# url-kaist/Quatro

Hardware: NVIDIA H100
Metric: registrations/sec (64-ring pair) (higher is better)
Workload: dtype f32 (front end, match, graph filter) / f64 (graph boundary, GNC, COTE)

## Files before the change

### quatro_b200/csrc/api.cu

```cuda
#include <new>
#include <stddef.h>
#include <stdio.h>
#include <stdlib.h>
#include <string.h>
#include <map>
#include <mutex>
#include <utility>

#include "handle.cuh"

using namespace qb;

namespace {

__global__ void wave_init_kernel(int* ctr_block, int n_ints, int* bbox, int n_clouds) {
  const int i = blockIdx.x * blockDim.x + threadIdx.x;
  if (i < n_ints) ctr_block[i] = 0;
  if (i < n_clouds * 6) bbox[i] = (i % 6) < 3 ? INT_MAX : INT_MIN;
}

__global__ void cache_copy_kernel(int to_cache, const int* __restrict__ slot_of_cloud, int V, float4* __restrict__ w_vox, float4* __restrict__ w_nrm,
                                  float* __restrict__ w_desc, int* __restrict__ w_n, int* __restrict__ w_status, float4* __restrict__ c_vox,
                                  float4* __restrict__ c_nrm, float* __restrict__ c_desc, int* __restrict__ c_n, int* __restrict__ c_status) {
  const int cloud = blockIdx.z, slot = slot_of_cloud[cloud], row = blockIdx.y;
  const int q = blockIdx.x * blockDim.x + threadIdx.x;
  if (slot < 0) return;
  const int n = to_cache ? w_n[cloud] : c_n[slot];
  if (row == 42) {
    if (q == 0) {
      if (to_cache) { c_n[slot] = w_n[cloud]; c_status[slot] = w_status[cloud]; }
      else { w_n[cloud] = c_n[slot]; w_status[cloud] = c_status[slot]; }
    }
    return;
  }
  if (q >= n || q >= V) return;
  if (row < kDescK) {
    float* w = w_desc + ((size_t)cloud * kDescK + row) * V + q;
    float* c = c_desc + ((size_t)slot * kDescK + row) * V + q;
    if (to_cache) *c = *w; else *w = *c;
  } else if (row == 40) {
    if (to_cache) c_vox[(size_t)slot * V + q] = w_vox[(size_t)cloud * V + q]; else w_vox[(size_t)cloud * V + q] = c_vox[(size_t)slot * V + q];
  } else {
    if (to_cache) c_nrm[(size_t)slot * V + q] = w_nrm[(size_t)cloud * V + q]; else w_nrm[(size_t)cloud * V + q] = c_nrm[(size_t)slot * V + q];
  }
}

size_t carve_counters(int* base, size_t S, WaveCounters* c) {
  const size_t C = 2 * S;
  size_t n = 0;
  auto take = [&](size_t k) {
    int* p = base ? base + n : nullptr;
    n += k;
    return p;
  };
  c->n_edges = reinterpret_cast<long long*>(take(2 * S));
  c->n_valid = take(C);
  c->n_vox = take(C);
  c->n_lat = take(C);
  c->n_cells = take(C);
  c->cloud_status = take(C);
  c->bbox = take(C * 6);
  c->vox_digits = take(C);
  c->n_mutual = take(S);
  c->n_corr = take(S);
  c->swapped = take(S);
  c->n_clique = take(S);
  c->max_core = take(S);
  c->n_final = take(S);
  c->flags = take(S);
  return n + 2;
}

int lane_alloc(const Lane& like, std::unique_ptr<Lane>* out) {
  std::unique_ptr<Lane> L(new (std::nothrow) Lane());
  if (!L) return QB200_ERR_CUDA;
  L->S = like.S; L->R = like.R; L->V = like.V; L->Lc = like.Lc; L->W = like.W; L->NS = like.NS;
  L->device = like.device; L->n_sm = like.n_sm; L->force_exact_match = like.force_exact_match; L->err = like.err;
  L->tc_verify = like.tc_verify; L->tc_prof = like.tc_prof;
  QB_CUDA_TRY(L, L->own_stream.create(cudaStreamNonBlocking));
  L->stream = L->own_stream;
  const size_t S = L->S, R = L->R, V = L->V, Lc = L->Lc, W = L->W, C = 2 * S;
  QB_CUDA_TRY(L, L->d_cloud_ptr.alloc(C));
  QB_CUDA_TRY(L, L->d_cloud_n.alloc(C));
  QB_CUDA_TRY(L, L->d_raw_off.alloc(C + 1));
  QB_CUDA_TRY(L, L->h_cloud_ptr.alloc(C));
  QB_CUDA_TRY(L, L->h_cloud_n.alloc(C));
  QB_CUDA_TRY(L, L->h_raw_off.alloc(C + 1));
  QB_CUDA_TRY(L, L->raw_stage.alloc(C * R));
  const size_t n_sort = C * (R > V ? R : V) + 64;
  const size_t n_hist = C * 256 * ((R + kVsTile - 1) / kVsTile);
  QB_CUDA_TRY(L, L->key_a.alloc(n_sort));
  QB_CUDA_TRY(L, L->key_b.alloc(n_sort));
  QB_CUDA_TRY(L, L->val_a.alloc(n_sort > n_hist ? n_sort : n_hist));
  QB_CUDA_TRY(L, L->val_b.alloc(n_sort));
  QB_CUDA_TRY(L, L->aos_scratch.alloc(2 * V * kDescDim));
  L->cub_bytes = sort_temp_bytes((int)(C * V));
  QB_CUDA_TRY(L, L->cub_temp.alloc_bytes(L->cub_bytes));
  QB_CUDA_TRY(L, L->vox_start.alloc(C * (V + 1)));
  QB_CUDA_TRY(L, L->vox_pts.alloc(C * V));
  QB_CUDA_TRY(L, L->cell_key.alloc(C * V));
  QB_CUDA_TRY(L, L->cell_start.alloc(C * (V + 1)));
  QB_CUDA_TRY(L, L->normals.alloc(C * V));
  QB_CUDA_TRY(L, L->spfh.alloc(C * V * kDescPad));
  QB_CUDA_TRY(L, L->nbr_list.alloc(C * kNbrGlobalCap * V));
  QB_CUDA_TRY(L, L->nbr_cnt.alloc(C * V));
  QB_CUDA_TRY(L, L->desc_t.alloc(C * kDescK * V));
  QB_CUDA_TRY(L, cudaMemset(L->desc_t, 0, C * kDescK * V * sizeof(float)));
  QB_CUDA_TRY(L, L->desc_tiles.alloc(C * kDescK * V * 3));
  QB_CUDA_TRY(L, cudaMemset(L->desc_tiles, 0, C * kDescK * V * 3 * sizeof(float)));
  QB_CUDA_TRY(L, L->desc_norm.alloc(C * V));
  QB_CUDA_TRY(L, L->tc_fallback.alloc(S));
  QB_CUDA_TRY(L, L->tc_stats.alloc(32));
  QB_CUDA_TRY(L, cudaMemset(L->tc_stats, 0, 32 * sizeof(unsigned long long)));
  QB_CUDA_TRY(L, L->rowbest.alloc(S * V));
  QB_CUDA_TRY(L, L->colpart.alloc(L->colpart_count()));
  QB_CUDA_TRY(L, L->colbest.alloc(S * V));
  QB_CUDA_TRY(L, L->mut_i.alloc(S * V));
  QB_CUDA_TRY(L, L->mut_j.alloc(S * V));
  QB_CUDA_TRY(L, L->mark.alloc(S * V));
  QB_CUDA_TRY(L, L->partner.alloc(S * V));
  QB_CUDA_TRY(L, L->mean.alloc(C * 4));
  QB_CUDA_TRY(L, L->corr_src.alloc(S * Lc));
  QB_CUDA_TRY(L, L->corr_tgt.alloc(S * Lc));
  QB_CUDA_TRY(L, L->ma.alloc(S * Lc));
  QB_CUDA_TRY(L, L->mb.alloc(S * Lc));
  QB_CUDA_TRY(L, L->adj.alloc(S * Lc * W));
  QB_CUDA_TRY(L, L->adjp.alloc(S * Lc * W));
  QB_CUDA_TRY(L, L->deg.alloc(S * Lc));
  QB_CUDA_TRY(L, L->kcore.alloc(S * (Lc + 2)));
  QB_CUDA_TRY(L, L->korder.alloc(S * (Lc + 2)));
  QB_CUDA_TRY(L, L->rank_of.alloc(S * (Lc + 2)));
  QB_CUDA_TRY(L, L->by_rank.alloc(S * (Lc + 2)));
  QB_CUDA_TRY(L, L->kbin.alloc(S * (Lc + 2)));
  QB_CUDA_TRY(L, L->clique.alloc(S * Lc));
  QB_CUDA_TRY(L, L->final_inl.alloc(S * Lc));
  QB_CUDA_TRY(L, L->rot_mask.alloc(S * Lc));
  QB_CUDA_TRY(L, L->trans_mask.alloc(S * Lc));
  QB_CUDA_TRY(L, L->d_solve.alloc(S));
  QB_CUDA_TRY(L, L->h_solve.alloc(S));
  QB_CUDA_TRY(L, L->d_front.alloc(C));
  QB_CUDA_TRY(L, L->h_front.alloc(C));
  if (Lc > (size_t)kKcoreSmemVerts) {
    QB_CUDA_TRY(L, L->kcore_ws.alloc(S * kcore_ws_bytes((int)Lc)));
    QB_CUDA_TRY(L, L->chain_ws.alloc(S * kCliqueWarps * Lc));
  }
  if (Lc > (size_t)kPoseSmemClique) QB_CUDA_TRY(L, L->pose_ws.alloc(S * pose_ws_bytes((int)Lc)));
  QB_CUDA_TRY(L, L->d_results.alloc(S));
  QB_CUDA_TRY(L, cudaMemset(L->d_results, 0, S * sizeof(qb200_result)));
  QB_CUDA_TRY(L, L->h_results.alloc(S));
  L->ctr_ints = carve_counters(nullptr, S, &L->ctr);
  QB_CUDA_TRY(L, L->ctr_block.alloc(L->ctr_ints));
  QB_CUDA_TRY(L, L->hctr_block.alloc(L->ctr_ints));
  carve_counters(L->ctr_block, S, &L->ctr);
  carve_counters(L->hctr_block, S, &L->hctr);
  for (Event& e : L->ev) QB_CUDA_TRY(L, e.create());
  for (Event& e : L->kev) QB_CUDA_TRY(L, e.create());
  QB_CUDA_TRY(L, cudaStreamSynchronize(L->stream));
  *out = std::move(L);
  return QB200_OK;
}

void reset_timers(qb200_handle* h) {
  memset(h->stage_ms, 0, sizeof(h->stage_ms));
  memset(h->kernel_ms, 0, sizeof(h->kernel_ms));
  memset(h->kernel_calls, 0, sizeof(h->kernel_calls));
}

}

namespace qb {
cudaError_t ensure_dyn_smem(int device, const void* kernel, size_t bytes) {
  static std::mutex mu;
  static std::map<std::pair<const void*, int>, size_t> current;
  std::lock_guard<std::mutex> lock(mu);
  size_t& cur = current[std::make_pair(kernel, device)];
  if (bytes > cur) {
    const cudaError_t e = cudaFuncSetAttribute(kernel, cudaFuncAttributeMaxDynamicSharedMemorySize, (int)bytes);
// ... 810 lines not shown
```

### quatro_b200/csrc/common.cuh

```cuda
#pragma once
#include <cuda_runtime.h>
#include <stdint.h>
#include <stdio.h>

#include "quatro_b200.h"

namespace qb {

constexpr int kOffIJ = 1 << 17;
constexpr int kOffK = 1 << 15;
constexpr uint64_t kCellMask = (1ull << 52) - 1;
constexpr uint64_t kCellInvalid = kCellMask;
constexpr int kCloudShift = 52;

__host__ __device__ __forceinline__ bool cell_ok(int i, int j, int k) {
  return i >= -kOffIJ && i < kOffIJ - 1 && j >= -kOffIJ && j < kOffIJ - 1 && k >= -kOffK && k < kOffK - 1;
}
__host__ __device__ __forceinline__ uint64_t cell_key(int i, int j, int k) {
  return ((uint64_t)(k + kOffK) << 36) | ((uint64_t)(j + kOffIJ) << 18) | (uint64_t)(i + kOffIJ);
}

constexpr int kVoxShift = 31;
constexpr uint64_t kVoxMask = (1ull << kVoxShift) - 1;
constexpr uint64_t kVoxInvalid = kVoxMask;
constexpr int kVsChunks = 64;
constexpr int kVsTile = 2048;

__device__ __forceinline__ bool raw_point_kept(const float4 p, int skip_flagged) {
  return isfinite(p.x) && isfinite(p.y) && isfinite(p.z) && !(skip_flagged && p.w < 0.0f);
}
__host__ __device__ __forceinline__ int vox_chunk_size(int n) { return n > 0 ? (n + kVsChunks - 1) / kVsChunks : 1; }

constexpr int kDescDim = 33;
constexpr int kDescPad = 36;
constexpr int kDescK = 40;
constexpr int kMatchTile = 128;
constexpr int kNbrGlobalCap = 80;

struct WaveCounters {
  int* n_valid;
  int* n_vox;
  int* n_lat;
  int* n_cells;
  int* cloud_status;
  int* bbox;
  int* vox_digits;
  int* n_mutual;
  int* n_corr;
  int* swapped;
  int* n_clique;
  int* max_core;
  int* n_final;
  int* flags;
  long long* n_edges;
};

#define QB_CUDA_TRY(h, expr)                                                                    \
  do {                                                                                          \
    cudaError_t _e = (expr);                                                                    \
    if (_e != cudaSuccess) {                                                                    \
      (h)->fail(__FILE__, __LINE__, cudaGetErrorString(_e));                                    \
      return QB200_ERR_CUDA;                                                                    \
    }                                                                                           \
  } while (0)

__device__ __forceinline__ int float_ordered(float f) {
  const int i = __float_as_int(f);
  return i >= 0 ? i : i ^ 0x7FFFFFFF;
}
__host__ __device__ __forceinline__ float ordered_float(int i) {
  const int j = i >= 0 ? i : i ^ 0x7FFFFFFF;
#ifdef __CUDA_ARCH__
  return __int_as_float(j);
#else
  float f;
  memcpy(&f, &j, 4);
  return f;
#endif
}

__host__ __device__ __forceinline__ bool vox_product_exceeds(long long a, long long b, long long c) {
  const long long lim = 2147483647LL;
  if (a > lim || b > lim || c > lim) return true;
  const long long ab = a * b;
  return ab > lim || ab * c > lim;
}
__device__ __forceinline__ bool vox_axis(int omin, int omax, float inv_leaf, long long* span, long long* min_b, long long* div_b) {
  const float mn = ordered_float(omin), mx = ordered_float(omax);
  const float lo = floorf(mn * inv_leaf), hi = floorf(mx * inv_leaf);
  if (!(lo >= -2147483648.0f && hi < 2147483648.0f)) return false;
  const float s = (mx - mn) * inv_leaf;
  if (!(s < 2147483648.0f)) return false;
  *span = (long long)s + 1;
  *min_b = (long long)lo;
  *div_b = (long long)hi - *min_b + 1;
  return true;
}
__device__ __forceinline__ bool vox_grid(const int* __restrict__ bbox, float inv_leaf, long long* min_b, long long* div_b) {
  long long t0, t1, t2;
  if (!vox_axis(bbox[0], bbox[3], inv_leaf, &t0, &min_b[0], &div_b[0]) || !vox_axis(bbox[1], bbox[4], inv_leaf, &t1, &min_b[1], &div_b[1]) ||
      !vox_axis(bbox[2], bbox[5], inv_leaf, &t2, &min_b[2], &div_b[2]))
    return false;
  return !vox_product_exceeds(t0, t1, t2) && !vox_product_exceeds(div_b[0], div_b[1], div_b[2]);
}

__device__ __forceinline__ int vox_digits(const int* __restrict__ bbox, int n_valid, float inv_leaf) {
  if (n_valid <= 0) return 0;
  long long m[3], d[3];
  if (!vox_grid(bbox, inv_leaf, m, d)) return -1;
// ... 40 lines not shown
```

### quatro_b200/csrc/frontend.cu

```cuda
#include <cub/device/device_radix_sort.cuh>
#include <type_traits>

#include "fpfh_math.cuh"
#include "handle.cuh"

namespace qb {

size_t sort_temp_bytes(int max_items) {
  size_t bytes = 0;
  cub::DeviceRadixSort::SortPairs(nullptr, bytes, (const uint64_t*)nullptr, (uint64_t*)nullptr, (const uint32_t*)nullptr,
                                  (uint32_t*)nullptr, max_items, 0, 64, (cudaStream_t)0);
  return bytes;
}

int sort_pairs(Lane* h, int n_items, int end_bit) {
  if (n_items <= 0) return QB200_OK;
  size_t bytes = h->cub_bytes;
  QB_CUDA_TRY(h, cub::DeviceRadixSort::SortPairs(h->cub_temp.get(), bytes, h->key_a.get(), h->key_b.get(), h->val_a.get(), h->val_b.get(), n_items, 0, end_bit,
                                                 h->stream));
  h->launches += 1 + (end_bit + 7) / 8;
  return QB200_OK;
}

static int clog2(int n) {
  int b = 0;
  while ((1 << b) < n) ++b;
  return b;
}


__global__ void __launch_bounds__(256) voxel_bbox_kernel(const float4* const* __restrict__ cloud_ptr, const int* __restrict__ cloud_n,
                                                         const CloudFront* __restrict__ front, int* __restrict__ bbox,
                                                         int* __restrict__ n_valid, int* __restrict__ chunk_cnt) {
  const int cloud = blockIdx.y;
  const int n = cloud_n[cloud];
  const int skip_flagged = front[cloud].skip_flagged;
  const float4* __restrict__ pts = cloud_ptr[cloud];
  int mn0 = INT_MAX, mn1 = INT_MAX, mn2 = INT_MAX, mx0 = INT_MIN, mx1 = INT_MIN, mx2 = INT_MIN, cnt = 0;
  constexpr int kInFlight = 8;
  __shared__ int s_cc[kVsChunks];
  if (threadIdx.x < kVsChunks) s_cc[threadIdx.x] = 0;
  __syncthreads();
  const int cs = vox_chunk_size(n);
  const int per_cta = kVsChunks / gridDim.x;
  for (int cl = 0; cl < per_cta; ++cl) {
    const int ch = blockIdx.x * per_cta + cl;
    const int c0 = ch * cs, c1 = min(n, c0 + cs);
    int ccnt = 0;
    for (int i0 = c0 + threadIdx.x; i0 < c1; i0 += kInFlight * 256) {
      float4 pp[kInFlight];
#pragma unroll
      for (int j = 0; j < kInFlight; ++j) pp[j] = i0 + j * 256 < c1 ? __ldg(pts + i0 + j * 256) : make_float4(NAN, NAN, NAN, 0.f);
#pragma unroll
      for (int j = 0; j < kInFlight; ++j) {
        const float4 p = pp[j];
        if (i0 + j * 256 >= c1 || !raw_point_kept(p, skip_flagged)) continue;
        const int ox = float_ordered(p.x), oy = float_ordered(p.y), oz = float_ordered(p.z);
        mn0 = min(mn0, ox); mn1 = min(mn1, oy); mn2 = min(mn2, oz);
        mx0 = max(mx0, ox); mx1 = max(mx1, oy); mx2 = max(mx2, oz);
        ++ccnt;
      }
    }
    cnt += ccnt;
    ccnt = __reduce_add_sync(0xffffffffu, ccnt);
    if (lane_id() == 0 && ccnt) atomicAdd(&s_cc[ch], ccnt);
  }
  __syncthreads();
  if ((int)threadIdx.x < per_cta) chunk_cnt[cloud * kVsChunks + blockIdx.x * per_cta + threadIdx.x] = s_cc[blockIdx.x * per_cta + threadIdx.x];
#pragma unroll
  for (int o = 16; o > 0; o >>= 1) {
    mn0 = min(mn0, __shfl_xor_sync(0xffffffffu, mn0, o)); mn1 = min(mn1, __shfl_xor_sync(0xffffffffu, mn1, o));
    mn2 = min(mn2, __shfl_xor_sync(0xffffffffu, mn2, o)); mx0 = max(mx0, __shfl_xor_sync(0xffffffffu, mx0, o));
    mx1 = max(mx1, __shfl_xor_sync(0xffffffffu, mx1, o)); mx2 = max(mx2, __shfl_xor_sync(0xffffffffu, mx2, o));
    cnt += __shfl_xor_sync(0xffffffffu, cnt, o);
  }
  __shared__ int s_red[7];
  if (threadIdx.x == 0) { s_red[0] = s_red[1] = s_red[2] = INT_MAX; s_red[3] = s_red[4] = s_red[5] = INT_MIN; s_red[6] = 0; }
  __syncthreads();
  if (lane_id() == 0 && cnt) {
    atomicMin(&s_red[0], mn0); atomicMin(&s_red[1], mn1); atomicMin(&s_red[2], mn2);
    atomicMax(&s_red[3], mx0); atomicMax(&s_red[4], mx1); atomicMax(&s_red[5], mx2);
    atomicAdd(&s_red[6], cnt);
  }
  __syncthreads();
  if (threadIdx.x == 0 && s_red[6]) {
    int* b = bbox + cloud * 6;
    atomicMin(b + 0, s_red[0]); atomicMin(b + 1, s_red[1]); atomicMin(b + 2, s_red[2]);
    atomicMax(b + 3, s_red[3]); atomicMax(b + 4, s_red[4]); atomicMax(b + 5, s_red[5]);
    atomicAdd(n_valid + cloud, s_red[6]);
  }
}

__global__ void __launch_bounds__(1024) run_heads_kernel(int mode, const uint64_t* keys, const uint64_t* keys_b, const int* __restrict__ seg_off,
                                                         int V, int key_shift, const CloudFront* __restrict__ front, const int* __restrict__ bbox,
                                                         const int* __restrict__ n_valid_in, int* __restrict__ starts,
                                                         uint64_t* __restrict__ cell_keys, int* __restrict__ n_out, int* __restrict__ n_valid_out,
                                                         int* __restrict__ cloud_status, int* __restrict__ digits_out) {
  __shared__ int sm[33];
  __shared__ int s_overflow, s_valid;
  const int cloud = blockIdx.x;
  const int off = mode == 0 ? seg_off[cloud] : cloud * V;
  const int n = mode == 0 ? n_valid_in[cloud] : V;
  const int digits = mode == 0 ? vox_digits(bbox + cloud * 6, n, front[cloud].inv_leaf) : 0;
  if (digits & 1) keys = keys_b;
  if (threadIdx.x == 0) {
    s_overflow = digits < 0 ? 1 : 0;
    s_valid = 0;
    if (digits_out) digits_out[cloud] = digits;
  }
  __syncthreads();
  if (s_overflow) {
    if (threadIdx.x == 0) {
      n_out[cloud] = 0;
      cloud_status[cloud] = QB200_ERR_VOXEL_OVERFLOW;
      starts[(size_t)cloud * (V + 1)] = 0;
    }
    return;
  }
// ... 412 lines not shown
__global__ void __launch_bounds__(kNbrThreads) fpfh_rare_kernel(const float4* __restrict__ pts, const int* __restrict__ n_pts, int V,
                                                                const uint64_t* __restrict__ cell_key, const int* __restrict__ cell_start,
                                                                const uint32_t* __restrict__ order, const int* __restrict__ n_cells,
                                                                const CloudFront* __restrict__ front, const float* __restrict__ spfh,
                                                                const int* __restrict__ nbr_cnt, float* __restrict__ desc_t) {
  const int cloud = blockIdx.y;
  const int q = blockIdx.x * blockDim.x + threadIdx.x;
  if (q >= n_pts[cloud]) return;
  if (nbr_cnt[(size_t)cloud * V + q] <= kNbrGlobalCap) return;
  const int m = front[cloud].mf;
  const float r2 = front[cloud].rf2;
  const LatticeView L = make_view(cloud, V, pts, cell_key, cell_start, order, n_cells, front[cloud].inv_cell);
  const float4* __restrict__ sp = reinterpret_cast<const float4*>(spfh + (size_t)cloud * V * kDescPad);
  const float4 pq = L.pts[q];
  float o[kDescDim];
#pragma unroll
  for (int b = 0; b < kDescDim; ++b) o[b] = 0.0f;
  double s0 = 0.0, s1 = 0.0, s2 = 0.0;
  for_each_neighbor<false>(L, pq, m, r2, [&](int p, float d2, const float4) {
    if (d2 == 0.0f) return;
    const float weight = 1.0f / d2;
    float s[kDescPad];
#pragma unroll
    for (int v4 = 0; v4 < kDescPad / 4; ++v4) {
      const float4 t = __ldg(sp + (size_t)p * (kDescPad / 4) + v4);
      s[4 * v4] = t.x; s[4 * v4 + 1] = t.y; s[4 * v4 + 2] = t.z; s[4 * v4 + 3] = t.w;
    }
#pragma unroll
    for (int b = 0; b < 11; ++b) { const float v = s[b] * weight; s0 += v; o[b] += v; }
#pragma unroll
    for (int b = 0; b < 11; ++b) { const float v = s[12 + b] * weight; s1 += v; o[11 + b] += v; }
#pragma unroll
    for (int b = 0; b < 11; ++b) { const float v = s[24 + b] * weight; s2 += v; o[22 + b] += v; }
  });
  if (s0 != 0.0) s0 = 100.0 / s0;
  if (s1 != 0.0) s1 = 100.0 / s1;
  if (s2 != 0.0) s2 = 100.0 / s2;
  const float g0 = (float)s0, g1 = (float)s1, g2 = (float)s2;
  float* __restrict__ out = desc_t + (size_t)cloud * kDescK * V + q;
#pragma unroll
  for (int b = 0; b < 11; ++b) out[(size_t)b * V] = o[b] * g0;
#pragma unroll
  for (int b = 11; b < 22; ++b) out[(size_t)b * V] = o[b] * g1;
#pragma unroll
  for (int b = 22; b < 33; ++b) out[(size_t)b * V] = o[b] * g2;
}

__global__ void desc_to_aos_kernel(const float* __restrict__ desc_t, int V, int n, float* __restrict__ out) {
  const int i = blockIdx.x * blockDim.x + threadIdx.x;
  if (i >= n * kDescDim) return;
  const int q = i / kDescDim, d = i % kDescDim;
  out[i] = desc_t[(size_t)d * V + q];
}
__global__ void desc_from_aos_kernel(const float* __restrict__ in, int V, int n, float* __restrict__ desc_t) {
  const int i = blockIdx.x * blockDim.x + threadIdx.x;
  if (i >= n * kDescDim) return;
  const int q = i / kDescDim, d = i % kDescDim;
  desc_t[(size_t)d * V + q] = in[i];
}

void front_voxel(CloudFront* e, float leaf, int skip_flagged) {
  e->inv_leaf = 1.0f / leaf;
  e->skip_flagged = skip_flagged;
}

void front_lattice(CloudFront* e, float normal_radius, float fpfh_radius, float cell) {
  e->inv_cell = 1.0f / cell;
  e->mn = (int)ceilf(normal_radius * e->inv_cell + 1e-3f);
  e->mf = (int)ceilf(fpfh_radius * e->inv_cell + 1e-3f);
  e->rn2 = (float)((double)normal_radius * (double)normal_radius);
  e->rf2 = (float)((double)fpfh_radius * (double)fpfh_radius);
  e->list_usable = (e->mn <= e->mf && e->rn2 <= e->rf2) ? 1 : 0;
}

int upload_front(Lane* L, int n) {
  QB_CUDA_TRY(L, cudaMemcpyAsync(L->d_front, L->h_front, (size_t)n * sizeof(CloudFront), cudaMemcpyHostToDevice, L->stream));
  return QB200_OK;
}

int launch_voxel(Lane* h, int n_clouds) {
  if (n_clouds <= 0) return QB200_OK;
  const dim3 gb(n_clouds >= 16 ? 16 : 64, n_clouds);
  int* chunk_cnt = reinterpret_cast<int*>(h->val_b.get());
  voxel_bbox_kernel<<<gb, 256, 0, h->stream>>>(h->d_cloud_ptr, h->d_cloud_n, h->d_front, h->ctr.bbox, h->ctr.n_valid, chunk_cnt);
  h->launches += 1;
  const int idx_bits = clog2(h->R > 2 ? h->R : 2);
  if (int rc = launch_voxel_sort(h, n_clouds, idx_bits)) return rc;
  run_heads_kernel<<<n_clouds, 1024, 0, h->stream>>>(0, h->key_a, h->key_b, h->d_raw_off, h->V, idx_bits, h->d_front, h->ctr.bbox, h->ctr.n_valid,
                                                     h->vox_start, nullptr, h->ctr.n_vox, nullptr, h->ctr.cloud_status, h->ctr.vox_digits);
  const dim3 gc((h->V + 127) / 128, n_clouds);
  voxel_centroid_kernel<<<gc, 128, 0, h->stream>>>(h->d_cloud_ptr, h->d_raw_off, h->key_a, h->key_b, h->ctr.vox_digits,
                                                   (1ull << idx_bits) - 1, h->vox_start, h->ctr.n_vox, h->V, h->vox_pts);
  h->launches += 2;
  QB_CUDA_TRY(h, cudaGetLastError());
  return QB200_OK;
}

int launch_fpfh(Lane* h, int n_clouds) {
  if (n_clouds <= 0) return QB200_OK;
  const int V = h->V;
  const dim3 gl((V + 255) / 256, n_clouds);
  lattice_keys_kernel<<<gl, 256, 0, h->stream>>>(h->vox_pts, h->ctr.n_vox, V, h->d_front, h->key_a, h->val_a);
  h->launches++;
  int rc = launch_cloud_sort(h, n_clouds, h->ctr.n_vox, 18, 36);
  if (rc == QB200_ERR_UNSUPPORTED) rc = sort_pairs(h, n_clouds * V, kCloudShift + clog2(n_clouds > 1 ? n_clouds : 2));
  if (rc) return rc;
  run_heads_kernel<<<n_clouds, 1024, 0, h->stream>>>(1, h->key_b, nullptr, nullptr, V, 0, nullptr, nullptr, nullptr, h->cell_start, h->cell_key,
                                                     h->ctr.n_cells, h->ctr.n_lat, h->ctr.cloud_status, nullptr);
  const dim3 gp((V + 127) / 128, n_clouds);
  nbr_list_kernel<<<gp, kNbrThreads, 0, h->stream>>>(h->vox_pts, h->ctr.n_vox, V, h->cell_key, h->cell_start, h->val_b, h->ctr.n_cells,
                                                     h->d_front, h->nbr_list, h->nbr_cnt);
  normals_kernel<<<gp, 128, 0, h->stream>>>(h->vox_pts, h->ctr.n_vox, V, h->cell_key, h->cell_start, h->val_b, h->ctr.n_cells, h->d_front,
                                            h->nbr_list, h->nbr_cnt, h->normals);
  spfh_kernel<false><<<gp, kSpfhThreads, 0, h->stream>>>(h->vox_pts, h->normals, h->ctr.n_vox, V, h->cell_key, h->cell_start, h->val_b,
                                                         h->ctr.n_cells, h->d_front, h->spfh, h->nbr_list, h->nbr_cnt);
  spfh_kernel<true><<<gp, kSpfhThreads, 0, h->stream>>>(h->vox_pts, h->normals, h->ctr.n_vox, V, h->cell_key, h->cell_start, h->val_b,
                                                        h->ctr.n_cells, h->d_front, h->spfh, h->nbr_list, h->nbr_cnt);
  fpfh_list_kernel<<<gp, 3 * kNbrThreads, 0, h->stream>>>(h->vox_pts, h->ctr.n_vox, V, h->spfh, h->nbr_list, h->nbr_cnt, h->desc_t);
  fpfh_rare_kernel<<<gp, kNbrThreads, 0, h->stream>>>(h->vox_pts, h->ctr.n_vox, V, h->cell_key, h->cell_start, h->val_b, h->ctr.n_cells,
                                                      h->d_front, h->spfh, h->nbr_cnt, h->desc_t);
  h->launches += 3;
  h->launches += 4;
  QB_CUDA_TRY(h, cudaGetLastError());
  return QB200_OK;
}

int launch_desc_to_aos(Lane* h, int cloud, int n, float* d_out33) {
  if (n <= 0) return QB200_OK;
  desc_to_aos_kernel<<<(n * kDescDim + 255) / 256, 256, 0, h->stream>>>(h->desc_t + (size_t)cloud * kDescK * h->V, h->V, n, d_out33);
  h->launches++;
  QB_CUDA_TRY(h, cudaGetLastError());
  return QB200_OK;
}
int desc_to_aos_rows(Lane* h, const float* desc_rows, int n, float* d_out33) {
  if (n <= 0) return QB200_OK;
  desc_to_aos_kernel<<<(n * kDescDim + 255) / 256, 256, 0, h->stream>>>(desc_rows, h->V, n, d_out33);
  h->launches++;
  QB_CUDA_TRY(h, cudaGetLastError());
  return QB200_OK;
}
int launch_desc_from_aos(Lane* h, int cloud, int n, const float* d_in33) {
  if (n <= 0) return QB200_OK;
  desc_from_aos_kernel<<<(n * kDescDim + 255) / 256, 256, 0, h->stream>>>(d_in33, h->V, n, h->desc_t + (size_t)cloud * kDescK * h->V);
  h->launches++;
  QB_CUDA_TRY(h, cudaGetLastError());
  return QB200_OK;
}

}
```

### quatro_b200/csrc/voxsort.cu

```cuda
#include "handle.cuh"

namespace qb {

constexpr int kVsThreads = 256;

__global__ void __launch_bounds__(kVsThreads) voxel_pack_kernel(const float4* const* __restrict__ cloud_ptr, const int* __restrict__ cloud_n,
                                                                const int* __restrict__ raw_off, const CloudFront* __restrict__ front,
                                                                const int* __restrict__ bbox, const int* __restrict__ n_valid,
                                                                const int* __restrict__ chunk_cnt, int idx_bits, uint64_t* __restrict__ items) {
  __shared__ int sm[33];
  const int cloud = blockIdx.y, chunk = blockIdx.x, tid = threadIdx.x;
  const int n = cloud_n[cloud], off = raw_off[cloud];
  const int cs = vox_chunk_size(n);
  const int c0 = chunk * cs, c1 = min(n, c0 + cs);
  if (c0 >= n) return;
  const float4* __restrict__ pts = cloud_ptr[cloud];
  const float inv_leaf = front[cloud].inv_leaf;
  const int skip_flagged = front[cloud].skip_flagged;
  long long m[3] = {0, 0, 0}, d[3] = {1, 1, 1};
  const bool grid_ok = n_valid[cloud] > 0 && vox_grid(bbox + cloud * 6, inv_leaf, m, d);
  int base = 0;
  {
    int v = 0;
    for (int k = tid; k < chunk; k += kVsThreads) v += chunk_cnt[cloud * kVsChunks + k];
    int tot;
    block_excl_scan(v, sm, &tot);
    base = tot;
  }
  constexpr int kPer = 4;
  for (int r0 = c0; r0 < c1; r0 += kPer * kVsThreads) {
    const int i0 = r0 + kPer * tid;
    uint64_t it[kPer];
    int keep[kPer], nk = 0;
#pragma unroll
    for (int j = 0; j < kPer; ++j) {
      const int i = i0 + j;
      keep[j] = 0; it[j] = 0;
      if (i < c1) {
        const float4 p = __ldg(pts + i);
        if (raw_point_kept(p, skip_flagged)) {
          uint64_t cell = kVoxInvalid;
          if (grid_ok) {
            const int ci = (int)floorf(p.x * inv_leaf), cj = (int)floorf(p.y * inv_leaf), ck = (int)floorf(p.z * inv_leaf);
            cell = (uint64_t)(((long long)ci - m[0]) + ((long long)cj - m[1]) * d[0] + ((long long)ck - m[2]) * d[0] * d[1]);
          }
          it[j] = (cell << idx_bits) | (uint64_t)i;
          keep[j] = 1;
        }
      }
      nk += keep[j];
    }
    int tot;
    int pos = base + block_excl_scan(nk, sm, &tot);
#pragma unroll
    for (int j = 0; j < kPer; ++j)
      if (keep[j]) items[off + pos++] = it[j];
    base += tot;
  }
}

__global__ void __launch_bounds__(kVsThreads) vsort_hist_kernel(int pass, const uint64_t* __restrict__ a, const uint64_t* __restrict__ b,
                                                                const int* __restrict__ raw_off, const int* __restrict__ bbox,
                                                                const int* __restrict__ n_valid, const CloudFront* __restrict__ front, int idx_bits,
                                                                int tiles_cap, unsigned* __restrict__ hist) {
  __shared__ unsigned s_h[256];
  const int cloud = blockIdx.y, tile = blockIdx.x, tid = threadIdx.x;
  const int m = n_valid[cloud];
  if (tile * kVsTile >= m || pass >= vox_digits(bbox + cloud * 6, m, front[cloud].inv_leaf)) return;
  const uint64_t* __restrict__ src = ((pass & 1) ? b : a) + raw_off[cloud];
  s_h[tid] = 0u;
  __syncthreads();
  const int shift = idx_bits + 8 * pass;
  const int t0 = tile * kVsTile, t1 = min(m, t0 + kVsTile);
  for (int i = t0 + tid; i < t1; i += kVsThreads) atomicAdd(&s_h[(unsigned)(src[i] >> shift) & 255u], 1u);
  __syncthreads();
  hist[((size_t)cloud * 256 + tid) * tiles_cap + tile] = s_h[tid];
}

__global__ void __launch_bounds__(1024) vsort_scan_kernel(int pass, const int* __restrict__ bbox, const int* __restrict__ n_valid,
                                                          const CloudFront* __restrict__ front, int tiles_cap, unsigned* __restrict__ hist) {
  __shared__ int sm[33];
  const int cloud = blockIdx.x, tid = threadIdx.x;
  const int m = n_valid[cloud];
  if (m <= 0 || pass >= vox_digits(bbox + cloud * 6, m, front[cloud].inv_leaf)) return;
  const int nt = (m + kVsTile - 1) / kVsTile;
  unsigned* __restrict__ H = hist + (size_t)cloud * 256 * tiles_cap;
  const int total = 256 * nt;
  int carry = 0;
  constexpr int kPer = 8;
  for (int base = 0; base < total; base += kPer * 1024) {
    const int e0 = base + kPer * tid;
    int v[kPer], s = 0;
#pragma unroll
    for (int j = 0; j < kPer; ++j) {
      const int e = e0 + j;
      v[j] = e < total ? (int)H[(size_t)(e / nt) * tiles_cap + (e % nt)] : 0;
      s += v[j];
    }
    int tot;
    int run = carry + block_excl_scan(s, sm, &tot);
#pragma unroll
    for (int j = 0; j < kPer; ++j) {
      const int e = e0 + j;
      if (e < total) H[(size_t)(e / nt) * tiles_cap + (e % nt)] = (unsigned)run;
      run += v[j];
    }
    carry += tot;
  }
}

__global__ void __launch_bounds__(kVsThreads) vsort_scatter_kernel(int pass, const uint64_t* __restrict__ a, const uint64_t* __restrict__ b,
                                                                   uint64_t* __restrict__ a_out, uint64_t* __restrict__ b_out,
                                                                   const int* __restrict__ raw_off, const int* __restrict__ bbox,
                                                                   const int* __restrict__ n_valid, const CloudFront* __restrict__ front,
                                                                   int idx_bits, int tiles_cap, const unsigned* __restrict__ offs) {
  __shared__ unsigned s_w[kVsThreads / 32][256];
  const int cloud = blockIdx.y, tile = blockIdx.x, tid = threadIdx.x, lane = tid & 31, warp = tid >> 5;
  const int m = n_valid[cloud];
  if (tile * kVsTile >= m || pass >= vox_digits(bbox + cloud * 6, m, front[cloud].inv_leaf)) return;
  const uint64_t* __restrict__ src = ((pass & 1) ? b : a) + raw_off[cloud];
  uint64_t* __restrict__ dst = ((pass & 1) ? a_out : b_out) + raw_off[cloud];
  const int shift = idx_bits + 8 * pass;
  const int t0 = tile * kVsTile + warp * 256;
#pragma unroll
  for (int k = 0; k < 8; ++k) s_w[warp][lane + 32 * k] = 0u;
  __syncwarp();
  uint64_t it[8];
  int dg[8];
#pragma unroll
  for (int r = 0; r < 8; ++r) {
    const int i = t0 + r * 32 + lane;
    dg[r] = -1 - lane;
    it[r] = 0;
    if (i < m) { it[r] = src[i]; dg[r] = (int)((unsigned)(it[r] >> shift) & 255u); }
    const unsigned peers = __match_any_sync(0xffffffffu, dg[r]);
    if (dg[r] >= 0 && (peers & ((1u << lane) - 1u)) == 0u) s_w[warp][dg[r]] += (unsigned)__popc(peers);
    __syncwarp();
  }
  __syncthreads();
  {
    unsigned run = offs[((size_t)cloud * 256 + tid) * tiles_cap + tile];
#pragma unroll
    for (int w = 0; w < kVsThreads / 32; ++w) {
      const unsigned c = s_w[w][tid];
      s_w[w][tid] = run;
      run += c;
    }
  }
  __syncthreads();
#pragma unroll
  for (int r = 0; r < 8; ++r) {
    const unsigned peers = __match_any_sync(0xffffffffu, dg[r]);
    if (dg[r] >= 0) {
      const unsigned rank = (unsigned)__popc(peers & ((1u << lane) - 1u));
      const unsigned pos = s_w[warp][dg[r]] + rank;
      dst[pos] = it[r];
    }
    __syncwarp();
    if (dg[r] >= 0 && (peers & ((1u << lane) - 1u)) == 0u) s_w[warp][dg[r]] += (unsigned)__popc(peers);
    __syncwarp();
  }
}

int launch_voxel_sort(Lane* h, int n_clouds, int idx_bits) {
  const int tiles_cap = (h->R + kVsTile - 1) / kVsTile;
  unsigned* hist = reinterpret_cast<unsigned*>(h->val_a.get());
  const int* chunk_cnt = reinterpret_cast<const int*>(h->val_b.get());
  const dim3 gp(kVsChunks, n_clouds), gt(tiles_cap, n_clouds);
  voxel_pack_kernel<<<gp, kVsThreads, 0, h->stream>>>(h->d_cloud_ptr, h->d_cloud_n, h->d_raw_off, h->d_front, h->ctr.bbox, h->ctr.n_valid,
                                                     chunk_cnt, idx_bits, h->key_a);
  for (int pass = 0; pass < 4; ++pass) {
    vsort_hist_kernel<<<gt, kVsThreads, 0, h->stream>>>(pass, h->key_a, h->key_b, h->d_raw_off, h->ctr.bbox, h->ctr.n_valid, h->d_front, idx_bits,
                                                       tiles_cap, hist);
    vsort_scan_kernel<<<n_clouds, 1024, 0, h->stream>>>(pass, h->ctr.bbox, h->ctr.n_valid, h->d_front, tiles_cap, hist);
    vsort_scatter_kernel<<<gt, kVsThreads, 0, h->stream>>>(pass, h->key_a, h->key_b, h->key_a, h->key_b, h->d_raw_off, h->ctr.bbox, h->ctr.n_valid,
                                                          h->d_front, idx_bits, tiles_cap, hist);
  }
  h->launches += 13;
  QB_CUDA_TRY(h, cudaGetLastError());
  return QB200_OK;
}

}
```

Measured before the change: 12900.

## Replace per-pass hist/scan/scatter radix sort with onesweep decoupled-lookback kernel

Voxel key radix sort changes from three kernels per pass (tile histogram, global scan, scatter) to one kernel per pass using decoupled lookback. Global digit histograms for all passes are built during the pack kernel, and status and counter words are zeroed in the bbox and pack kernels. Each tile takes a dynamic tile index, publishes its aggregate and inclusive prefix with relaxed stores, spins on its predecessors, then stages items in shared memory for more coalesced scatter writes. This cuts launches from 13 to 5 and removes the extra histogram read of the keys. In exchange it depends on spin-wait forward progress, has a spin-limit failure path, and raises shared memory use per block.

After: 13090, median of 6. 1.5% higher.

```diff
diff --git a/quatro_b200/csrc/api.cu b/quatro_b200/csrc/api.cu
--- a/quatro_b200/csrc/api.cu
+++ b/quatro_b200/csrc/api.cu
@@ -88,11 +88,12 @@
   QB_CUDA_TRY(L, L->h_raw_off.alloc(C + 1));
   QB_CUDA_TRY(L, L->raw_stage.alloc(C * R));
   const size_t n_sort = C * (R > V ? R : V) + 64;
-  const size_t n_hist = C * 256 * ((R + kVsTile - 1) / kVsTile);
+  const size_t n_status = C * 256 * ((R + kVsTile - 1) / kVsTile);
+  const size_t n_vs_ctr = C * (kVsChunks + kVsCtrWords);
   QB_CUDA_TRY(L, L->key_a.alloc(n_sort));
   QB_CUDA_TRY(L, L->key_b.alloc(n_sort));
-  QB_CUDA_TRY(L, L->val_a.alloc(n_sort > n_hist ? n_sort : n_hist));
-  QB_CUDA_TRY(L, L->val_b.alloc(n_sort));
+  QB_CUDA_TRY(L, L->val_a.alloc(n_sort > n_status ? n_sort : n_status));
+  QB_CUDA_TRY(L, L->val_b.alloc(n_sort > n_vs_ctr ? n_sort : n_vs_ctr));
   QB_CUDA_TRY(L, L->aos_scratch.alloc(2 * V * kDescDim));
   L->cub_bytes = sort_temp_bytes((int)(C * V));
   QB_CUDA_TRY(L, L->cub_temp.alloc_bytes(L->cub_bytes));
diff --git a/quatro_b200/csrc/common.cuh b/quatro_b200/csrc/common.cuh
--- a/quatro_b200/csrc/common.cuh
+++ b/quatro_b200/csrc/common.cuh
@@ -25,6 +25,7 @@
 constexpr uint64_t kVoxInvalid = kVoxMask;
 constexpr int kVsChunks = 64;
 constexpr int kVsTile = 2048;
+constexpr int kVsCtrWords = 4 * 256 + 4;
 
 __device__ __forceinline__ bool raw_point_kept(const float4 p, int skip_flagged) {
   return isfinite(p.x) && isfinite(p.y) && isfinite(p.z) && !(skip_flagged && p.w < 0.0f);
diff --git a/quatro_b200/csrc/frontend.cu b/quatro_b200/csrc/frontend.cu
--- a/quatro_b200/csrc/frontend.cu
+++ b/quatro_b200/csrc/frontend.cu
@@ -31,9 +31,11 @@
 
 __global__ void __launch_bounds__(256) voxel_bbox_kernel(const float4* const* __restrict__ cloud_ptr, const int* __restrict__ cloud_n,
                                                          const CloudFront* __restrict__ front, int* __restrict__ bbox,
-                                                         int* __restrict__ n_valid, int* __restrict__ chunk_cnt) {
+                                                         int* __restrict__ n_valid, int* __restrict__ chunk_cnt, unsigned* __restrict__ vs_ctr) {
   const int cloud = blockIdx.y;
   const int n = cloud_n[cloud];
+  if (blockIdx.x == 0)
+    for (int k = threadIdx.x; k < kVsCtrWords; k += blockDim.x) vs_ctr[cloud * kVsCtrWords + k] = 0u;
   const int skip_flagged = front[cloud].skip_flagged;
   const float4* __restrict__ pts = cloud_ptr[cloud];
   int mn0 = INT_MAX, mn1 = INT_MAX, mn2 = INT_MAX, mx0 = INT_MIN, mx1 = INT_MIN, mx2 = INT_MIN, cnt = 0;
@@ -612,7 +614,8 @@
   if (n_clouds <= 0) return QB200_OK;
   const dim3 gb(n_clouds >= 16 ? 16 : 64, n_clouds);
   int* chunk_cnt = reinterpret_cast<int*>(h->val_b.get());
-  voxel_bbox_kernel<<<gb, 256, 0, h->stream>>>(h->d_cloud_ptr, h->d_cloud_n, h->d_front, h->ctr.bbox, h->ctr.n_valid, chunk_cnt);
+  voxel_bbox_kernel<<<gb, 256, 0, h->stream>>>(h->d_cloud_ptr, h->d_cloud_n, h->d_front, h->ctr.bbox, h->ctr.n_valid, chunk_cnt,
+                                               h->val_b.get() + (size_t)n_clouds * kVsChunks);
   h->launches += 1;
   const int idx_bits = clog2(h->R > 2 ? h->R : 2);
   if (int rc = launch_voxel_sort(h, n_clouds, idx_bits)) return rc;
diff --git a/quatro_b200/csrc/voxsort.cu b/quatro_b200/csrc/voxsort.cu
--- a/quatro_b200/csrc/voxsort.cu
+++ b/quatro_b200/csrc/voxsort.cu
@@ -3,14 +3,36 @@
 namespace qb {
 
 constexpr int kVsThreads = 256;
+constexpr int kVsSpinLimit = 400000;
+
+constexpr unsigned kVsAggregate = 1u;
+constexpr unsigned kVsInclusive = 2u;
+constexpr unsigned kVsCountMask = (1u << 28) - 1u;
+
+__device__ __forceinline__ void vs_publish(unsigned* p, unsigned flag, int pass, unsigned count) {
+  asm volatile("st.relaxed.gpu.global.u32 [%0], %1;" ::"l"(p), "r"(flag << 30 | (unsigned)pass << 28 | count) : "memory");
+}
+__device__ __forceinline__ unsigned vs_poll(const unsigned* p) {
+  unsigned v;
+  asm volatile("ld.relaxed.gpu.global.u32 %0, [%1];" : "=r"(v) : "l"(p) : "memory");
+  return v;
+}
 
 __global__ void __launch_bounds__(kVsThreads) voxel_pack_kernel(const float4* const* __restrict__ cloud_ptr, const int* __restrict__ cloud_n,
                                                                 const int* __restrict__ raw_off, const CloudFront* __restrict__ front,
                                                                 const int* __restrict__ bbox, const int* __restrict__ n_valid,
-                                                                const int* __restrict__ chunk_cnt, int idx_bits, uint64_t* __restrict__ items) {
+                                                                const int* __restrict__ chunk_cnt, int idx_bits, int tiles_cap,
+                                                                uint64_t* __restrict__ items, unsigned* __restrict__ hist,
+                                                                unsigned* __restrict__ status) {
   __shared__ int sm[33];
+  __shared__ unsigned s_h[4 * 256];
   const int cloud = blockIdx.y, chunk = blockIdx.x, tid = threadIdx.x;
-  const int n = cloud_n[cloud], off = raw_off[cloud];
+  const int n = cloud_n[cloud], off = raw_off[cloud], nv = n_valid[cloud];
+  {
+    unsigned* __restrict__ st = status + (size_t)cloud * tiles_cap * 256;
+    const int words = (nv + kVsTile - 1) / kVsTile * 256;
+    for (int w = chunk * kVsThreads + tid; w < words; w += kVsChunks * kVsThreads) st[w] = 0u;
+  }
   const int cs = vox_chunk_size(n);
   const int c0 = chunk * cs, c1 = min(n, c0 + cs);
   if (c0 >= n) return;
@@ -18,7 +40,9 @@
   const float inv_leaf = front[cloud].inv_leaf;
   const int skip_flagged = front[cloud].skip_flagged;
   long long m[3] = {0, 0, 0}, d[3] = {1, 1, 1};
-  const bool grid_ok = n_valid[cloud] > 0 && vox_grid(bbox + cloud * 6, inv_leaf, m, d);
+  const bool grid_ok = nv > 0 && vox_grid(bbox + cloud * 6, inv_leaf, m, d);
+  const int digits = grid_ok ? vox_digits(bbox + cloud * 6, nv, inv_leaf) : 0;
+  for (int k = tid; k < 4 * 256; k += kVsThreads) s_h[k] = 0u;
   int base = 0;
   {
     int v = 0;
@@ -44,6 +68,7 @@
             const int ci = (int)floorf(p.x * inv_leaf), cj = (int)floorf(p.y * inv_leaf), ck = (int)floorf(p.z * inv_leaf);
             cell = (uint64_t)(((long long)ci - m[0]) + ((long long)cj - m[1]) * d[0] + ((long long)ck - m[2]) * d[0] * d[1]);
           }
+          for (int g = 0; g < digits; ++g) atomicAdd(&s_h[g * 256 + ((unsigned)(cell >> (8 * g)) & 255u)], 1u);
           it[j] = (cell << idx_bits) | (uint64_t)i;
           keep[j] = 1;
         }
@@ -57,126 +82,120 @@
       if (keep[j]) items[off + pos++] = it[j];
     base += tot;
   }
-}
-
-__global__ void __launch_bounds__(kVsThreads) vsort_hist_kernel(int pass, const uint64_t* __restrict__ a, const uint64_t* __restrict__ b,
-                                                                const int* __restrict__ raw_off, const int* __restrict__ bbox,
-                                                                const int* __restrict__ n_valid, const CloudFront* __restrict__ front, int idx_bits,
-                                                                int tiles_cap, unsigned* __restrict__ hist) {
-  __shared__ unsigned s_h[256];
-  const int cloud = blockIdx.y, tile = blockIdx.x, tid = threadIdx.x;
+  __syncthreads();
+  for (int k = tid; k < digits * 256; k += kVsThreads)
+    if (s_h[k]) atomicAdd(&hist[cloud * kVsCtrWords + k], s_h[k]);
+}
+
+__global__ void __launch_bounds__(kVsThreads, 5) vsort_onesweep_kernel(int pass, const uint64_t* __restrict__ a, const uint64_t* __restrict__ b,
+                                                                    uint64_t* __restrict__ a_out, uint64_t* __restrict__ b_out,
+                                                                    const int* __restrict__ raw_off, const int* __restrict__ bbox,
+                                                                    int* __restrict__ n_valid, const CloudFront* __restrict__ front,
+                                                                    int idx_bits, int tiles_cap, unsigned* __restrict__ ctr,
+                                                                    unsigned* __restrict__ status, int* __restrict__ cloud_status) {
+  __shared__ unsigned s_w[kVsThreads / 32][256];
+  __shared__ uint64_t s_it[kVsTile];
+  __shared__ int s_off[256];
+  __shared__ int sm[33];
+  __shared__ int s_tile, s_fail;
+  const int cloud = blockIdx.x, tid = threadIdx.x, lane = tid & 31, warp = tid >> 5;
   const int m = n_valid[cloud];
-  if (tile * kVsTile >= m || pass >= vox_digits(bbox + cloud * 6, m, front[cloud].inv_leaf)) return;
-  const uint64_t* __restrict__ src = ((pass & 1) ? b : a) + raw_off[cloud];
-  s_h[tid] = 0u;
-  __syncthreads();
-  const int shift = idx_bits + 8 * pass;
-  const int t0 = tile * kVsTile, t1 = min(m, t0 + kVsTile);
-  for (int i = t0 + tid; i < t1; i += kVsThreads) atomicAdd(&s_h[(unsigned)(src[i] >> shift) & 255u], 1u);
-  __syncthreads();
-  hist[((size_t)cloud * 256 + tid) * tiles_cap + tile] = s_h[tid];
-}
-
-__global__ void __launch_bounds__(1024) vsort_scan_kernel(int pass, const int* __restrict__ bbox, const int* __restrict__ n_valid,
-                                                          const CloudFront* __restrict__ front, int tiles_cap, unsigned* __restrict__ hist) {
-  __shared__ int sm[33];
-  const int cloud = blockIdx.x, tid = threadIdx.x;
-  const int m = n_valid[cloud];
-  if (m <= 0 || pass >= vox_digits(bbox + cloud * 6, m, front[cloud].inv_leaf)) return;
-  const int nt = (m + kVsTile - 1) / kVsTile;
-  unsigned* __restrict__ H = hist + (size_t)cloud * 256 * tiles_cap;
-  const int total = 256 * nt;
-  int carry = 0;
-  constexpr int kPer = 8;
-  for (int base = 0; base < total; base += kPer * 1024) {
-    const int e0 = base + kPer * tid;
-    int v[kPer], s = 0;
-#pragma unroll
-    for (int j = 0; j < kPer; ++j) {
-      const int e = e0 + j;
-      v[j] = e < total ? (int)H[(size_t)(e / nt) * tiles_cap + (e % nt)] : 0;
-      s += v[j];
-    }
-    int tot;
-    int run = carry + block_excl_scan(s, sm, &tot);
-#pragma unroll
-    for (int j = 0; j < kPer; ++j) {
-      const int e = e0 + j;
-      if (e < total) H[(size_t)(e / nt) * tiles_cap + (e % nt)] = (unsigned)run;
-      run += v[j];
-    }
-    carry += tot;
-  }
-}
-
-__global__ void __launch_bounds__(kVsThreads) vsort_scatter_kernel(int pass, const uint64_t* __restrict__ a, const uint64_t* __restrict__ b,
-                                                                   uint64_t* __restrict__ a_out, uint64_t* __restrict__ b_out,
-                                                                   const int* __restrict__ raw_off, const int* __restrict__ bbox,
-                                                                   const int* __restrict__ n_valid, const CloudFront* __restrict__ front,
-                                                                   int idx_bits, int tiles_cap, const unsigned* __restrict__ offs) {
-  __shared__ unsigned s_w[kVsThreads / 32][256];
-  const int cloud = blockIdx.y, tile = blockIdx.x, tid = threadIdx.x, lane = tid & 31, warp = tid >> 5;
-  const int m = n_valid[cloud];
-  if (tile * kVsTile >= m || pass >= vox_digits(bbox + cloud * 6, m, front[cloud].inv_leaf)) return;
+  if ((int)blockIdx.y * kVsTile >= m || pass >= vox_digits(bbox + cloud * 6, m, front[cloud].inv_leaf)) return;
+  unsigned* __restrict__ cc = ctr + (size_t)cloud * kVsCtrWords;
+  if (tid == 0) {
+    s_tile = (int)atomicAdd(cc + 4 * 256 + pass, 1u);
+    s_fail = 0;
+  }
+#pragma unroll
+  for (int k = 0; k < 8; ++k) s_w[warp][lane + 32 * k] = 0u;
+  __syncthreads();
+  const int tile = s_tile;
   const uint64_t* __restrict__ src = ((pass & 1) ? b : a) + raw_off[cloud];
   uint64_t* __restrict__ dst = ((pass & 1) ? a_out : b_out) + raw_off[cloud];
   const int shift = idx_bits + 8 * pass;
   const int t0 = tile * kVsTile + warp * 256;
-#pragma unroll
-  for (int k = 0; k < 8; ++k) s_w[warp][lane + 32 * k] = 0u;
-  __syncwarp();
   uint64_t it[8];
   int dg[8];
 #pragma unroll
   for (int r = 0; r < 8; ++r) {
     const int i = t0 + r * 32 + lane;
-    dg[r] = -1 - lane;
-    it[r] = 0;
-    if (i < m) { it[r] = src[i]; dg[r] = (int)((unsigned)(it[r] >> shift) & 255u); }
+    it[r] = i < m ? __ldg(src + i) : 0;
+  }
+#pragma unroll
+  for (int r = 0; r < 8; ++r) dg[r] = t0 + r * 32 + lane < m ? (int)((unsigned)(it[r] >> shift) & 255u) : -1 - lane;
+#pragma unroll
+  for (int r = 0; r < 8; ++r) {
     const unsigned peers = __match_any_sync(0xffffffffu, dg[r]);
     if (dg[r] >= 0 && (peers & ((1u << lane) - 1u)) == 0u) s_w[warp][dg[r]] += (unsigned)__popc(peers);
     __syncwarp();
   }
   __syncthreads();
-  {
-    unsigned run = offs[((size_t)cloud * 256 + tid) * tiles_cap + tile];
-#pragma unroll
-    for (int w = 0; w < kVsThreads / 32; ++w) {
-      const unsigned c = s_w[w][tid];
-      s_w[w][tid] = run;
-      run += c;
+  unsigned agg = 0;
+#pragma unroll
+  for (int w = 0; w < kVsThreads / 32; ++w) {
+    const unsigned c = s_w[w][tid];
+    s_w[w][tid] = agg;
+    agg += c;
+  }
+  unsigned* __restrict__ st = status + (size_t)cloud * tiles_cap * 256 + tid;
+  vs_publish(st + 256 * tile, tile == 0 ? kVsInclusive : kVsAggregate, pass, agg);
+  unsigned excl = 0;
+  for (int j = tile - 1; j >= 0; --j) {
+    unsigned v = 0;
+    for (int spin = 0; spin < kVsSpinLimit; ++spin) {
+      v = vs_poll(st + 256 * j);
+      if ((v >> 30) != 0u && ((v >> 28) & 3u) == (unsigned)pass) break;
     }
-  }
+    if ((v >> 30) == 0u || ((v >> 28) & 3u) != (unsigned)pass) { s_fail = 1; break; }
+    excl += v & kVsCountMask;
+    if ((v >> 30) == kVsInclusive) break;
+  }
+  if (tile > 0) vs_publish(st + 256 * tile, kVsInclusive, pass, excl + agg);
+  int tot;
+  const int gbase = block_excl_scan((int)cc[256 * pass + tid], sm, &tot);
+  const int lbase = block_excl_scan((int)agg, sm, &tot);
+  s_off[tid] = gbase + (int)excl - lbase;
+#pragma unroll
+  for (int w = 0; w < kVsThreads / 32; ++w) s_w[w][tid] += (unsigned)lbase;
   __syncthreads();
 #pragma unroll
   for (int r = 0; r < 8; ++r) {
     const unsigned peers = __match_any_sync(0xffffffffu, dg[r]);
-    if (dg[r] >= 0) {
-      const unsigned rank = (unsigned)__popc(peers & ((1u << lane) - 1u));
-      const unsigned pos = s_w[warp][dg[r]] + rank;
-      dst[pos] = it[r];
-    }
+    if (dg[r] >= 0) s_it[s_w[warp][dg[r]] + (unsigned)__popc(peers & ((1u << lane) - 1u))] = it[r];
     __syncwarp();
     if (dg[r] >= 0 && (peers & ((1u << lane) - 1u)) == 0u) s_w[warp][dg[r]] += (unsigned)__popc(peers);
     __syncwarp();
   }
+  __syncthreads();
+  if (s_fail) {
+    if (tid == 0) {
+      cloud_status[cloud] = QB200_ERR_CUDA;
+      n_valid[cloud] = 0;
+    }
+    return;
+  }
+  const int cnt = min(kVsTile, m - tile * kVsTile);
+  for (int i = tid; i < cnt; i += kVsThreads) {
+    const uint64_t v = s_it[i];
+    const int pos = s_off[(unsigned)(v >> shift) & 255u] + i;
+    if ((unsigned)pos < (unsigned)m) dst[pos] = v;
+  }
 }
 
 int launch_voxel_sort(Lane* h, int n_clouds, int idx_bits) {
   const int tiles_cap = (h->R + kVsTile - 1) / kVsTile;
-  unsigned* hist = reinterpret_cast<unsigned*>(h->val_a.get());
+  unsigned* status = h->val_a.get();
   const int* chunk_cnt = reinterpret_cast<const int*>(h->val_b.get());
-  const dim3 gp(kVsChunks, n_clouds), gt(tiles_cap, n_clouds);
+  unsigned* ctr = h->val_b.get() + (size_t)n_clouds * kVsChunks;
+  int max_n = 1;
+  for (int c = 0; c < n_clouds; ++c) max_n = max(max_n, h->h_cloud_n[c]);
+  const dim3 gp(kVsChunks, n_clouds), gt(n_clouds, (max_n + kVsTile - 1) / kVsTile);
   voxel_pack_kernel<<<gp, kVsThreads, 0, h->stream>>>(h->d_cloud_ptr, h->d_cloud_n, h->d_raw_off, h->d_front, h->ctr.bbox, h->ctr.n_valid,
-                                                     chunk_cnt, idx_bits, h->key_a);
-  for (int pass = 0; pass < 4; ++pass) {
-    vsort_hist_kernel<<<gt, kVsThreads, 0, h->stream>>>(pass, h->key_a, h->key_b, h->d_raw_off, h->ctr.bbox, h->ctr.n_valid, h->d_front, idx_bits,
-                                                       tiles_cap, hist);
-    vsort_scan_kernel<<<n_clouds, 1024, 0, h->stream>>>(pass, h->ctr.bbox, h->ctr.n_valid, h->d_front, tiles_cap, hist);
-    vsort_scatter_kernel<<<gt, kVsThreads, 0, h->stream>>>(pass, h->key_a, h->key_b, h->key_a, h->key_b, h->d_raw_off, h->ctr.bbox, h->ctr.n_valid,
-                                                          h->d_front, idx_bits, tiles_cap, hist);
-  }
-  h->launches += 13;
+                                                     chunk_cnt, idx_bits, tiles_cap, h->key_a, ctr, status);
+  for (int pass = 0; pass < 4; ++pass)
+    vsort_onesweep_kernel<<<gt, kVsThreads, 0, h->stream>>>(pass, h->key_a, h->key_b, h->key_a, h->key_b, h->d_raw_off, h->ctr.bbox,
+                                                           h->ctr.n_valid, h->d_front, idx_bits, tiles_cap, ctr, status, h->ctr.cloud_status);
+  h->launches += 5;
   QB_CUDA_TRY(h, cudaGetLastError());
   return QB200_OK;
 }
```
